# SunYangtian/Splatter_A_Video

Measured on AMD Instinct MI355X. Metric: rendered frames/sec fwd+bwd @480p, 300k Gaussians, higher is better.
Workload: dtype f32

## Files before the change

include/splat_hip.h:

```cpp
#ifndef SPLAT_HIP_H
#define SPLAT_HIP_H

#include <stddef.h>
#include <stdint.h>

#ifdef __cplusplus
extern "C" {
#endif

typedef void *splat_stream_t;

#define SPLAT_OK 0
#define SPLAT_E_ARG (-1)
#define SPLAT_E_LAUNCH (-2)
#define SPLAT_E_CAPACITY (-3)

const char *splat_last_error(void);
#define SPLAT_ABI_VERSION 22
int splat_abi_version(void);
const char *splat_build_id(void);
void splat_set_deterministic(int on);
int splat_get_deterministic(void);
int splat_fill_f32(float *dst, size_t n, float value, splat_stream_t stream);
int splat_set_option(const char *key, int value);
// ... 175 lines not shown
                                         float nearest, float extent, float *uv, float *depth, float *conic,
                                         int32_t *radius, splat_stream_t stream);
int splat_bin_count_batch(int F, int P, const float *uv, const int32_t *radius, int W, int H, void *scratch,
                          int32_t *tile_range, int32_t *M_out, splat_stream_t stream);
int splat_bin_sort_batch(int F, int P, const float *uv, const float *depth, const int32_t *radius, int W, int H,
                         void *scratch, int32_t *tile_range, int64_t capacity, uint64_t *keys, int32_t *idx_sorted,
                         int32_t *overflow_out, int32_t *goff_incl , int32_t *owner, int32_t *slot_sorted,
                         splat_stream_t stream);
int splat_bin_count_batch_reach(int F, int P, const float *uv, const int32_t *radius, const float *conic,
                                const float *opacity, int64_t opacity_frame_stride, int W, int H, void *scratch,
                                int32_t *tile_range, int32_t *M_out, int32_t *gcount, uint32_t *reach, splat_stream_t stream);
int splat_bin_sort_batch_reach(int F, int P, const float *uv, const float *depth, const int32_t *radius, const uint32_t *reach,
                               int W, int H, void *scratch, int32_t *tile_range, int64_t capacity, uint64_t *keys,
                               int32_t *idx_sorted, int32_t *overflow_out, int32_t *goff_incl , int32_t *owner,
                               int32_t *slot_sorted, splat_stream_t stream);
int splat_alpha_blending_forward_batch(int F, int P, int C, const float *uv, const float *conic, const float *opacity,
                                       int64_t opacity_frame_stride, const float *feature, int64_t feature_frame_stride,
                                       const int32_t *idx_sorted, const int32_t *tile_range, int64_t capacity, float bg,
                                       const float *bg_channels, int W, int H, int K, int enable_truncation, float *out,
                                       float *final_T, int32_t *ncontrib, int32_t *gs_idx, float *pack_scratch,
                                       uint32_t *cull_flags , splat_stream_t stream);
size_t splat_blend_pair_stride(int C, int want_abs, int has_bias);
int splat_alpha_blending_backward_batch(int F, int P, int C, const int32_t *idx_sorted, const int32_t *tile_range,
                                        int64_t capacity, float bg, int W, int H, const float *final_T,
                                        const int32_t *ncontrib, const float *dL_dout, int want_abs,
                                        const int32_t *slot_sorted, float *pair_records, const float *pack,
                                        const uint32_t *cull_flags ,
                                        float *dbg_T_front , splat_stream_t stream);
int splat_frames_gauss_backward_static(int F, int P, int C, int W, int H, int64_t capacity, int want_abs,
                                       const float *pair_records, const int32_t *goff_incl, const int32_t *radius,
                                       const float *xyz, const float *scales, const float *uquats, const float *extr,
                                       int accumulate, float *d_xyz, float *d_scales, float *d_uquats, float *d_opacity,
                                       float *d_feature, float *tap, float *abs_tap, int32_t *radii_max,
                                       splat_stream_t stream);

typedef struct splat_camera_t {
// ... 249 lines not shown
```

splatter_a_video_amd/_lib.py:

```python
from __future__ import annotations

import ctypes
import os
from typing import Optional

import torch

_HERE = os.path.dirname(os.path.abspath(__file__))
LIB_PATH = os.environ.get("SPLAT_LIB_PATH") or os.path.join(_HERE, "libsplat_hip.so")
_lib: Optional[ctypes.CDLL] = None

ABI_VERSION = 22

SYMBOLS = [
    "splat_last_error", "splat_abi_version", "splat_build_id", "splat_set_deterministic", "splat_get_deterministic",
    "splat_fill_f32", "splat_set_option", "splat_get_option",
    "splat_project_point_forward", "splat_project_point_backward",
    "splat_compute_cov3d_forward", "splat_compute_cov3d_backward",
    "splat_ewa_project_forward", "splat_ewa_project_backward",
    "splat_compute_sh_forward", "splat_compute_sh_backward",
    "splat_bin_scratch_bytes", "splat_bin_count", "splat_bin_sort",
    "splat_compute_gaussian_key", "splat_compute_tile_gaussian_range",
    "splat_alpha_blending_forward", "splat_alpha_blending_backward", "splat_alpha_blending_forward_flags",
    "splat_alpha_blending_backward_flags", "splat_blend_pair_floats", "splat_blend_pack_floats",
# ... 13 lines not shown
    "splat_frames_gauss_backward_static", "splat_alpha_blending_backward_batch_set", "splat_frames_gauss_backward_static_set",
    "splat_blend_sets_pair_stride", "splat_blend_sets_pack_floats", "splat_alpha_blending_backward_batch_sets",
    "splat_alpha_blending_forward_batch_sets", "splat_pair_records_segment_sum", "splat_alpha_blending_backward_batch_sets_packed",
    "splat_frames_gauss_backward_static_sets", "splat_frames_gauss_backward_dynamic_sets",
    "splat_preprocess_forward_batch_cam", "splat_frames_gauss_backward_static_cam", "splat_frames_gauss_backward_static_sets_cam",
    "splat_preprocess_persp_forward", "splat_preprocess_persp_backward",
    "splat_alpha_blending_forward_batch_sources", "splat_frames_gauss_backward_dynamic_sources",
    "splat_frames_gauss_backward_static_sources_cam", "splat_blend_sets_uses_forward_pack",
    "splat_dynamic_positions_batch_forward", "splat_dynamic_positions_batch_backward",
    "splat_arap_energy_batch", "splat_knn_brute_scratch_bytes", "splat_knn_brute_batch", "splat_l1_loss_grad",
    "splat_alpha_blending_backward_batch_sets_l1", "splat_bin_count_batch_reach", "splat_bin_sort_batch_reach",
    "splat_profile_enable", "splat_profile_reset", "splat_profile_read",
    "splat_ssim_scratch_bytes", "splat_ssim_forward", "splat_ssim_backward", "splat_dssim_l1_loss_grad",
    "splat_track_loss_scratch_bytes", "splat_track_loss_grad",
    "splat_depth_dpt_scratch_bytes", "splat_depth_stats", "splat_depth_dpt_loss_grad",
]


class SplatError(RuntimeError):
    pass


_raw_stream = getattr(torch._C, "_cuda_getCurrentRawStream", None)
_cur_device = getattr(torch._C, "_cuda_getDevice", None)


def lib() -> ctypes.CDLL:
    global _lib
    if _lib is None:
        if not os.path.exists(LIB_PATH):
# ... 147 lines not shown
```

splatter_a_video_amd/csrc/binning.hip:

```cpp
#include "common.h"
#include <cstdlib>

#define BIN_BLOCK 256
#define BIN_MAX_NB 512
#define BIN_CHUNK 512
#define BIN_CHUNK_BATCH 2048
#define BIN_BATCH_FRAMES 4
#define BIN_LDS_TILES 12288
#define BIN_GLOBAL_BLOCKS 2048
#define SORT_BLOCK 256
#define SORT_LDS_KEYS 2048

struct BinPlan {
    int T, gx, gy;
    int NB;
    int chunk;
    bool lds;
    int nchunk;
    size_t off_matrix, off_tilecount, off_total, off_chunksum;
    size_t bytes;
};

static inline int imax(int a, int b) { return a > b ? a : b; }
static inline int imin(int a, int b) { return a < b ? a : b; }
// ... 48 lines not shown
__device__ __forceinline__ int reach_cell_shift(int w, int h) {
    int sh = 1;
    while ((((w - 1) >> sh) + 1) * (((h - 1) >> sh) + 1) > 31) ++sh;
    return sh;
}
__device__ __forceinline__ int reach_big_count(unsigned word, int w, int h) {
    const int sh = reach_cell_shift(w, h), c = 1 << sh, ncx = ((w - 1) >> sh) + 1, ncy = ((h - 1) >> sh) + 1;
    int n = 0;
    unsigned bit = 1u;
    for (int cy = 0; cy < ncy; ++cy)
        for (int cx = 0; cx < ncx; ++cx, bit <<= 1)
            if (word & bit) n += imin_(c, w - cx * c) * imin_(c, h - cy * c);
    return n;
}

template <bool LDS>
__global__ void __launch_bounds__(BIN_BLOCK)
bin_count_kernel(int P, const float2 *__restrict__ uv, const int *__restrict__ radius, int gx, int gy, int T,
                 int chunk, int *__restrict__ matrix, int *__restrict__ gcount, int *__restrict__ chunk_sum,
                 long long S, const float *__restrict__ conic, const float *__restrict__ opacity, long long opacity_fs,
                 unsigned *__restrict__ reach) {
    extern __shared__ __attribute__((aligned(16))) int cnt[];
    __shared__ int wave_pairs[BIN_BLOCK / 64];
    const int wg = blockIdx.x;
    {
        const size_t f = blockIdx.y;
        uv += f * P; radius += f * P; matrix += f * S; chunk_sum += f * S;
        if (gcount) gcount += f * P;
        if (reach) { conic += f * 3 * (size_t)P; opacity += f * (size_t)opacity_fs; reach += f * P; }
    }
    int pairs = 0;
    if (LDS) {
        for (int t = threadIdx.x; t < T; t += BIN_BLOCK) cnt[t] = 0;
        __syncthreads();
    }
    const int beg = wg * chunk, end = imin_(P, beg + chunk);
    for (int i = beg + threadIdx.x; i < end; i += BIN_BLOCK) {
        const int r = radius[i];
        if (r <= 0) {
            if (gcount) gcount[i] = 0;
            if (reach) reach[i] = 0u;
            continue;
        }
        const float2 q = uv[i];
        int x0, y0, x1, y1;
        tile_rect(q.x, q.y, r, gx, gy, x0, y0, x1, y1);
        const int area = (x1 - x0) * (y1 - y0);
        if (reach) {
            const float cA = conic[3 * (size_t)i], cB = conic[3 * (size_t)i + 1], cC = conic[3 * (size_t)i + 2], o = opacity[i];
            unsigned word;
            int kept = 0;
            if (area < 32) {
                const CullP cp = cull_params(cA, cB, cC, o);
                unsigned m = 0u, bit = 1u;
                for (int ty = y0; ty < y1; ++ty)
                    for (int tx = x0; tx < x1; ++tx, bit <<= 1) {
                        const float fx = (float)(tx * TILE), fy = (float)(ty * TILE);
                        if (cull_test(q.x, q.y, cA, cB, cC, cp, fx, fx + (float)(TILE - 1), fy, fy + (float)(TILE - 1))) {
                            m |= bit;
                            if (LDS) atomicAdd(&cnt[ty * gx + tx], 1);
                            else atomicAdd(&matrix[ty * gx + tx], 1);
                        }
                    }
                kept = __popc(m);
                word = m;
            } else {
// ... 555 lines not shown
                idx_sorted[r0 + i] = id;
            } else {
                idx_sorted[r0 + i] = (int)lo;
            }
        }
    }
}

extern "C" size_t splat_bin_scratch_bytes(int P, int W, int H) {
    if (P < 0 || W <= 0 || H <= 0) return 0;
    return make_plan(P, W, H).bytes;
}

static int bin_count_impl(int F, int P, const float *uv, const int32_t *radius, int W, int H, void *scratch,
                          int32_t *tile_range, int32_t *M_out, int32_t *gcount, hipStream_t s, const float *conic = nullptr,
                          const float *opacity = nullptr, long long opacity_fs = 0, uint32_t *reach = nullptr) {
    const BinPlan p = make_plan(P, W, H, F);
    const long long S = (long long)(p.bytes / sizeof(int));
    char *base = (char *)scratch;
    int *matrix = (int *)(base + p.off_matrix);
    int *tile_count = (int *)(base + p.off_tilecount);
    int *total = (int *)(base + p.off_total);
    int *chunk_sum = (int *)(base + p.off_chunksum);
    if (p.lds) {
        SPLAT_LAUNCH("bin_count", bin_count_kernel<true>, dim3(p.NB, F), dim3(BIN_BLOCK), (size_t)p.T * sizeof(int), s,
                     P, (const float2 *)uv, radius, p.gx, p.gy, p.T, p.chunk, matrix, gcount, chunk_sum, S, conic, opacity, opacity_fs,
                     reach);
    } else {
        for (int f = 0; f < F; ++f)
            SPLAT_CHECK_HIP(hipMemsetAsync(matrix + (size_t)f * S, 0, (size_t)p.T * sizeof(int), s));
        const int nblk = p.nchunk;
        const int chunk = (P + nblk - 1) / nblk;
        SPLAT_LAUNCH("bin_count", bin_count_kernel<false>, dim3(nblk, F), dim3(BIN_BLOCK), 0, s, P, (const float2 *)uv,
                     radius, p.gx, p.gy, p.T, chunk > 0 ? chunk : 1, matrix, gcount, chunk_sum, S, conic, opacity, opacity_fs, reach);
    }
    SPLAT_POST_LAUNCH();
    if (p.lds) {
        SPLAT_LAUNCH("bin_colscan", bin_colscan_kernel, dim3((p.T + COLSCAN_COLS - 1) / COLSCAN_COLS, F),
                     dim3(COLSCAN_COLS * COLSCAN_GROUPS), 0, s, p.T, p.NB, matrix, tile_count, S);
        SPLAT_POST_LAUNCH();
    } else {
        for (int f = 0; f < F; ++f)
            SPLAT_CHECK_HIP(hipMemcpyAsync(tile_count + (size_t)f * S, matrix + (size_t)f * S, (size_t)p.T * sizeof(int),
                                           hipMemcpyDeviceToDevice, s));
    }
    SPLAT_LAUNCH("bin_tilescan", bin_tilescan_kernel, dim3(1, F), dim3(1024), 0, s, p.T, tile_count, tile_range, M_out, total,
                 p.nchunk, chunk_sum, S);
    SPLAT_POST_LAUNCH();
    return SPLAT_OK;
}
// ... 71 lines not shown
    return bin_sort_impl(F, P, uv, depth, radius, W, H, scratch, tile_range, capacity, keys, idx_sorted, overflow_out,
                         goff_incl, owner_scratch, slot_sorted, (hipStream_t)stream);
}


extern "C" int splat_bin_count_batch_reach(int F, int P, const float *uv, const int32_t *radius, const float *conic,
                                           const float *opacity, int64_t opacity_frame_stride, int W, int H, void *scratch,
                                           int32_t *tile_range, int32_t *M_out, int32_t *gcount, uint32_t *reach,
                                           splat_stream_t stream) {
    SPLAT_CHECK_ARG(F >= 1 && F <= 65535 && P >= 1 && W > 0 && H > 0 && opacity_frame_stride >= 0, "bad sizes");
    SPLAT_CHECK_ARG(scratch && tile_range && uv && radius && conic && opacity && reach, "null pointer");
    return bin_count_impl(F, P, uv, radius, W, H, scratch, tile_range, M_out, gcount, (hipStream_t)stream, conic, opacity,
                          (long long)opacity_frame_stride, reach);
}

extern "C" int splat_bin_sort_batch_reach(int F, int P, const float *uv, const float *depth, const int32_t *radius,
                                          const uint32_t *reach, int W, int H, void *scratch, int32_t *tile_range,
                                          int64_t capacity, uint64_t *keys, int32_t *idx_sorted, int32_t *overflow_out,
                                          int32_t *goff_incl, int32_t *owner_scratch, int32_t *slot_sorted,
                                          splat_stream_t stream) {
    SPLAT_CHECK_ARG(F >= 1 && F <= 65535 && P >= 1 && W > 0 && H > 0 && capacity >= 1, "bad sizes");
    SPLAT_CHECK_ARG(scratch && tile_range && overflow_out && uv && depth && radius && keys && idx_sorted && goff_incl &&
                        owner_scratch && slot_sorted && reach,
                    "null pointer");
    return bin_sort_impl(F, P, uv, depth, radius, W, H, scratch, tile_range, capacity, keys, idx_sorted, overflow_out,
                         goff_incl, owner_scratch, slot_sorted, (hipStream_t)stream, reach);
}


__global__ void __launch_bounds__(256)
// ... 59 lines not shown
```

splatter_a_video_amd/csrc/blend.hip:

```cpp
#include <stdlib.h>

#include <utility>

#include "common.h"

__device__ __forceinline__ float exp2_guard(float pw, bool &ok) {
    ok = true;
    return __builtin_amdgcn_fmed3f(__builtin_amdgcn_exp2f(pw), 0.f, 1.f);
}

struct BlendArgs {
    int P, C;
    int c0, cn;
    const float2 *uv;
    const float *conic;
    const float *opacity;
    const float *feature;
    const float *bias;
    const int *idx_sorted;
    const int2 *tile_range;
    float bg;
    const float *bgc;
    int W, H, gx;
    int K, trunc;
// ... 92 lines not shown
    pw = __builtin_fmaf(xx, c0.w, pw);
    pw = __builtin_fmaf(xy, c1.x, pw);
    return __builtin_fmaf(yy, c1.y, pw);
}
__device__ __forceinline__ float neg_power_factored(float dx, float dy, float cA, float cB, float cC) {
#pragma clang fp contract(off)
    const float h = __builtin_fmaf(cA, 0.5f * dx, cB * dy);
    return __builtin_fmaf(dx, h, (cC * (0.5f * dy)) * dy);
}
__device__ __forceinline__ float exp_neg(float q) { return __builtin_amdgcn_exp2f(-BLEND_L2E * q); }

struct __attribute__((packed, aligned(4))) F3 {
    float x, y, z;
};

template <int CH>
struct Rec {
    static constexpr int RS = (8 + CH + 15) & ~15;
    static constexpr int RQ = RS / 4;
    static constexpr int CULL = (RS - 8 - CH >= 5) ? RS - 5 : -1;
};


template <bool SETS = false>
__device__ __forceinline__ void stage_feature_rows(float *s_rec, int LS, int at, const float *src, int cn, int i0, int nrec) {
    if (!src || cn <= 0) return;
    const float *p = src + (size_t)i0 * cn;
    for (int e = threadIdx.x; e < nrec * cn; e += 256) {
        const int row = e / cn, ch = e - row * cn;
        s_rec[row * LS + (SETS ? 8 + 8 * ((at + ch) & 3) + ((at + ch) >> 2) : at + ch)] = p[e];
    }
}

template <int CH, bool BIAS, bool EXACT>
__global__ void __launch_bounds__(256)
pack_kernel(const BlendArgs B) {
    const BlendArgs A = frame_args(B, blockIdx.y);
    constexpr int RS = Rec<CH>::RS, RQ = Rec<CH>::RQ;
    constexpr int LS = RS + 4;
    __shared__ __attribute__((aligned(16))) float s_rec[256 * LS];
    const int i0 = blockIdx.x * 256;
    const int i = i0 + threadIdx.x;
    float r[RS];
#pragma unroll
    for (int k = 0; k < RS; ++k) r[k] = 0.f;
    if (i < A.P) {
        const float2 q = A.uv[i];
        r[0] = q.x; r[1] = q.y;
        r[2] = A.conic[3 * i]; r[3] = A.conic[3 * i + 1]; r[4] = A.conic[3 * i + 2];
        r[5] = A.opacity[i];
        if (BIAS) r[6] = A.bias[i];
        r[7] = __int_as_float(i);
        if (A.feature) {
            const float *f = A.feature + (size_t)i * A.C + A.c0;
#pragma unroll
            for (int k = 0; k < CH; ++k)
                if (EXACT || k < A.cn) r[8 + k] = f[k];
        }
        if (Rec<CH>::CULL >= 0) {
            constexpr int CO = Rec<CH>::CULL >= 0 ? Rec<CH>::CULL : 0;
            const CullP cp = cull_params(r[2], r[3], r[4], r[5]);
            r[CO] = cp.hx; r[CO + 1] = cp.hy; r[CO + 2] = cp.tauq; r[CO + 3] = cp.ia; r[CO + 4] = cp.ic;
        }
    }
    {
        float4 *row = reinterpret_cast<float4 *>(s_rec + threadIdx.x * LS);
#pragma unroll
        for (int k = 0; k < RS; k += 4) row[k / 4] = make_float4(r[k], r[k + 1], r[k + 2], r[k + 3]);
        __syncthreads();
        const int nrec = imin_(256, A.P - i0);
        if (!A.feature) {
            for (int sidx = 0; sidx < B.nsrc; ++sidx)
                stage_feature_rows(s_rec, LS, 8 + B.src_c0[sidx] - B.c0, B.src_f[sidx] + (size_t)blockIdx.y * B.src_fs[sidx],
                                   B.src_cn[sidx], i0, nrec);
            __syncthreads();
        }
        float4 *dst = reinterpret_cast<float4 *>(A.pack + (size_t)i0 * RS);
        for (int c = threadIdx.x; c < nrec * RQ; c += 256) {
// ... 3235 lines not shown
template <int CH>
static int launch_pack(const BlendArgs &A, bool bias, hipStream_t s) {
    if (A.P == 0) return SPLAT_OK;
    const dim3 grid((unsigned)((A.P + 255) / 256), (unsigned)A.F), block(256);
    const bool exact = A.cn == CH;
    if (bias) { if (exact) SPLAT_LAUNCH("blend_pack", (pack_kernel<CH, true, true>), grid, block, 0, s, A); else SPLAT_LAUNCH("blend_pack", (pack_kernel<CH, true, false>), grid, block, 0, s, A); }
    else { if (exact) SPLAT_LAUNCH("blend_pack", (pack_kernel<CH, false, true>), grid, block, 0, s, A); else SPLAT_LAUNCH("blend_pack", (pack_kernel<CH, false, false>), grid, block, 0, s, A); }
    SPLAT_POST_LAUNCH();
    return SPLAT_OK;
}

template <int CH>
static int launch_fwd(const BlendArgs &A, int T, bool enh, bool bias, hipStream_t s) {
    const dim3 grid((unsigned)(T * A.F)), block(256);
    const bool exact = A.cn == CH;
    {
        const int rc = launch_pack<CH>(A, bias, s);
        if (rc != SPLAT_OK) return rc;
    }
#define FWD(E, B, X) SPLAT_LAUNCH("blend_fwd", (blend_fwd_kernel<CH, E, B, X>), grid, block, 0, s, A)
    if (enh) {
        if (bias) { if (exact) FWD(true, true, true); else FWD(true, true, false); }
        else { if (exact) FWD(true, false, true); else FWD(true, false, false); }
    } else {
        if (bias) { if (exact) FWD(false, true, true); else FWD(false, true, false); }
        else { if (exact) FWD(false, false, true); else FWD(false, false, false); }
    }
#undef FWD
    SPLAT_POST_LAUNCH();
    return SPLAT_OK;
}
// ... 35 lines not shown
        SPLAT_POST_LAUNCH();
    }
    return SPLAT_OK;
}

template <int CH>
static int launch_bwd(const BlendArgs &A, int T, bool bias, bool pair, hipStream_t s) {
    if (!A.pack_valid) {
        const int rc = launch_pack<CH>(A, bias, s);
        if (rc != SPLAT_OK) return rc;
    }
    const bool abs_ = A.dL_dabs_uv != nullptr;
    if (abs_) return bias ? launch_bwd_ab<CH, true, true>(A, T, pair, s) : launch_bwd_ab<CH, true, false>(A, T, pair, s);
    return bias ? launch_bwd_ab<CH, false, true>(A, T, pair, s) : launch_bwd_ab<CH, false, false>(A, T, pair, s);
}

static inline int chunk_ch(int cn) { return cn <= 1 ? 1 : cn <= 3 ? 3 : cn <= 8 ? 8 : cn <= 16 ? 16 : cn <= 20 ? 20 : cn <= 24 ? 24 : 32; }

static int fwd_chunk(const BlendArgs &A, int T, bool enh, bool bias, hipStream_t s) {
    switch (chunk_ch(A.cn)) {
        case 1: return launch_fwd<1>(A, T, enh, bias, s);
        case 3: return launch_fwd<3>(A, T, enh, bias, s);
        case 8: return launch_fwd<8>(A, T, enh, bias, s);
        case 16: return launch_fwd<16>(A, T, enh, bias, s);
        case 20: return launch_fwd<20>(A, T, enh, bias, s);
        case 24: return launch_fwd<24>(A, T, enh, bias, s);
        default: return launch_fwd<32>(A, T, enh, bias, s);
    }
}

static int bwd_chunk(const BlendArgs &A, int T, bool bias, bool pair, hipStream_t s) {
    switch (chunk_ch(A.cn)) {
// ... 144 lines not shown
                                                   const int32_t *slot_sorted, float *pair_scratch, float *pack_scratch,
                                                   int pack_is_valid, float *dbg_T_front, const uint32_t *cull_flags,
                                                   splat_stream_t stream) {
    return blend_backward_impl(P, C, uv, conic, opacity, feature, opacity_bias, idx_sorted, tile_range, bg, W, H, final_T, ncontrib,
                               dL_dout, dL_duv, dL_dabs_uv, dL_dconic, dL_dopacity, dL_dfeature, dL_dopacity_bias, dL_dndc,
                               dL_dabs_ndc, goff_incl, slot_sorted, pair_scratch, pack_scratch, pack_is_valid, dbg_T_front,
                               cull_flags, stream);
}


extern "C" size_t splat_blend_pair_stride(int C, int want_abs, int has_bias) {
    const int ng = 6 + (want_abs ? 2 : 0) + (has_bias ? 1 : 0);
    return (size_t)PAIR_STRIDE(ng + chunk_ch(C > 32 ? 32 : C));
}

extern "C" int splat_alpha_blending_forward_batch(int F, int P, int C, const float *uv, const float *conic,
                                                  const float *opacity, int64_t opacity_frame_stride,
                                                  const float *feature, int64_t feature_frame_stride,
                                                  const int32_t *idx_sorted, const int32_t *tile_range, int64_t capacity,
                                                  float bg, const float *bg_channels, int W, int H, int K,
                                                  int enable_truncation, float *out, float *final_T, int32_t *ncontrib,
                                                  int32_t *gs_idx, float *pack_scratch, uint32_t *cull_flags,
                                                  splat_stream_t stream) {
    SPLAT_CHECK_ARG(F >= 1 && P >= 1 && C >= 1 && C <= 32 && W > 0 && H > 0 && capacity >= 1, "bad sizes (C <= 32)");
    SPLAT_CHECK_ARG(uv && conic && opacity && feature && idx_sorted && tile_range && out && final_T && ncontrib &&
                        pack_scratch,
                    "null pointer");
    const bool enh = (gs_idx != nullptr) && K > 0;
    BlendArgs A;
    memset(&A, 0, sizeof(A));
    A.P = P; A.C = C;
    A.uv = (const float2 *)uv; A.conic = conic; A.opacity = opacity; A.feature = feature;
    A.idx_sorted = idx_sorted; A.tile_range = (const int2 *)tile_range;
    A.bg = bg; A.bgc = bg_channels; A.W = W; A.H = H; A.gx = (W + TILE - 1) / TILE;
    A.K = enh ? K : 0; A.trunc = enable_truncation ? 1 : 0;
    A.out = out; A.final_T = final_T; A.ncontrib = ncontrib; A.gs_idx = gs_idx;
    A.pack = pack_scratch;
    A.cull_flags = cull_flags;
    const int T = A.gx * ((H + TILE - 1) / TILE);
    SPLAT_CHECK_ARG((long long)F * T < (1ll << 31), "too many tiles");
    A.F = F; A.T = T; A.cap = capacity;
    A.pack_fs = (long long)P * (long long)splat_blend_pack_floats(C);
    A.opacity_fs = opacity_frame_stride; A.feature_fs = feature_frame_stride;
    A.c0 = 0; A.cn = C;
    return fwd_chunk(A, T, enh, false, (hipStream_t)stream);
}

extern "C" int splat_alpha_blending_forward_batch_sources(int F, int P, int C, int nsrc, const splat_feature_source_t *src,
                                                          const float *uv, const float *conic, const float *opacity,
                                                          int64_t opacity_frame_stride, const int32_t *idx_sorted,
                                                          const int32_t *tile_range, int64_t capacity,
                                                          const float *bg_channels, int W, int H, int K, int enable_truncation,
                                                          float *out, float *final_T, int32_t *ncontrib, int32_t *gs_idx,
                                                          float *pack_scratch, uint32_t *cull_flags, splat_stream_t stream) {
    SPLAT_CHECK_ARG(F >= 1 && P >= 1 && C >= 1 && C <= 32 && W > 0 && H > 0 && capacity >= 1, "bad sizes (C <= 32)");
    SPLAT_CHECK_ARG(src && nsrc >= 1 && nsrc <= SPLAT_MAX_SOURCES && bg_channels, "null / oversized source table");
    SPLAT_CHECK_ARG(uv && conic && opacity && idx_sorted && tile_range && out && final_T && ncontrib && pack_scratch, "null pointer");
    BlendArgs A;
    memset(&A, 0, sizeof(A));
    {
// ... 324 lines not shown
```

splatter_a_video_amd/csrc/common.h:

```cpp
#pragma once
#include <hip/hip_runtime.h>
#include <stdint.h>
#include <stdio.h>
#include <string.h>

#include "../../include/splat_hip.h"

#define TILE 16
#define TILE_PIX 256
#define WAVE 64

void splat_set_error(const char *fmt, ...);

#define SPLAT_CHECK_ARG(cond, msg)                     \
    do {                                               \
        if (!(cond)) {                                 \
            splat_set_error("%s: %s", __func__, msg);  \
            return SPLAT_E_ARG;                        \
        }                                              \
    } while (0)

#define SPLAT_CHECK_HIP(expr)                                                          \
    do {                                                                               \
        hipError_t e_ = (expr);                                                        \
// ... 87 lines not shown
    const float t = 255.f * o;
    if (t < 0.999f) {
        p.hx = -1.f;
        return p;
    }
    const float det = a * c - b * b;
    if (!(det > 0.f) || !(a > 0.f) || !(c > 0.f)) return p;
    const float relerr = 4e-7f * (a * c + b * b) / det;
    if (!(relerr < 0.25f)) return p;
    const float tau0 = fmaxf(2.f * __logf(t), 0.f);
    const float tau = tau0 * (1.f + 2.f * relerr) * 1.002f + 2e-3f;
    const float inv = 1.f / det;
    p.hx = sqrtf(tau * c * inv) * 1.001f + 0.01f;
    p.hy = sqrtf(tau * a * inv) * 1.001f + 0.01f;
    p.tauq = tau * 1.002f + 2e-3f;
    p.ia = 1.f / a;
    p.ic = 1.f / c;
    return p;
}

__device__ __forceinline__ bool cull_test(float u, float v, float a, float b, float c, const CullP &p, float bx0,
                                          float bx1, float by0, float by1) {
    const float dx0 = bx0 - u, dx1 = bx1 - u, dy0 = by0 - v, dy1 = by1 - v;
    const float ddx = fmaxf(fmaxf(dx0, -dx1), 0.f);
    const float ddy = fmaxf(fmaxf(dy0, -dy1), 0.f);
    if (!((ddx <= p.hx) && (ddy <= p.hy))) return false;
    if (ddx == 0.f && ddy == 0.f) return true;
    const float INF = __builtin_inff();
    const float xe = dx0 > 0.f ? dx0 : dx1, ye = dy0 > 0.f ? dy0 : dy1;
    const float ys = fminf(fmaxf(-b * xe * p.ic, dy0), dy1), xs = fminf(fmaxf(-b * ye * p.ia, dx0), dx1);
    const float qx = a * xe * xe + 2.f * b * xe * ys + c * ys * ys;
    const float qy = a * xs * xs + 2.f * b * xs * ye + c * ye * ye;
    const float qmin = fminf(ddx > 0.f ? qx : INF, ddy > 0.f ? qy : INF);
    const float r2 = fmaxf(dx0 * dx0, dx1 * dx1) + fmaxf(dy0 * dy0, dy1 * dy1);
    const float qerr = 4e-6f * (a + c + 2.f * fabsf(b)) * r2;
    return qmin <= p.tauq + qerr;
}

template <bool ABS, bool BIAS>
struct GradLayout {
    static constexpr int NG = 6 + (ABS ? 2 : 0) + (BIAS ? 1 : 0);
    static constexpr int I_ABS = 6;
    static constexpr int I_BIAS = 6 + (ABS ? 2 : 0);
};
#define PAIR_STRIDE(nc) (((nc) + 3) & ~3)
constexpr int SETS_NG = 12;
constexpr int XCD_RUN = 64;
__device__ __forceinline__ int xcd_tile(int b, int T) {
    constexpr int S = XCD_RUN;
    const int full = (T / (8 * S)) * (8 * S);
    if (b >= full) return b;
    const int x = b & 7, q = b >> 3;
    return ((q / S) * 8 + x) * S + (q % S);
// ... 4 lines not shown
```

splatter_a_video_amd/csrc/frames.hip:

```cpp
#include "common.h"

static splat_camera_t batch_camera(const splat_frames_t *b) {
    splat_camera_t cam;
    memset(&cam, 0, sizeof(cam));
    cam.perspective = b->perspective; cam.intr = b->intr; cam.intr_frame_stride = b->intr_frame_stride;
    cam.extr = b->extr; cam.extr_frame_stride = b->extr_frame_stride; cam.offsets = b->offsets;
    return cam;
}

static int frames_bin_count(const splat_frames_t *b) {
    if (b->reach) {
        SPLAT_CHECK_ARG(b->opacity != nullptr, "reach masks need the opacity");
        return splat_bin_count_batch_reach(b->F, b->P, b->uv, b->radius, b->conic, b->opacity, 0, b->W, b->H, b->bin_scratch,
                                           b->tile_range, b->pairs, nullptr, b->reach, b->stream);
    }
    return splat_bin_count_batch(b->F, b->P, b->uv, b->radius, b->W, b->H, b->bin_scratch, b->tile_range, b->pairs, b->stream);
}

extern "C" int splat_frames_forward(const splat_frames_t *b) {
    SPLAT_CHECK_ARG(b != nullptr && b->struct_bytes == sizeof(splat_frames_t), "splat_frames_t of another ABI version");
    SPLAT_CHECK_ARG(b->capacity >= 1, "capacity (pairs reserved per frame) must be set: run splat_frames_count first");
    const splat_camera_t cam = batch_camera(b);
    int rc = splat_preprocess_forward_batch_cam(b->F, b->P, b->xyz, b->offsets, b->scales, b->uquats, &cam, b->W, b->H,
                                                b->nearest, b->extent, b->uv, b->depth, b->conic, b->radius, b->stream);
    if (rc != SPLAT_OK) return rc;
    rc = frames_bin_count(b);
    if (rc != SPLAT_OK) return rc;
    if (b->reach)
        rc = splat_bin_sort_batch_reach(b->F, b->P, b->uv, b->depth, b->radius, b->reach, b->W, b->H, b->bin_scratch,
                                        b->tile_range, b->capacity, b->keys, b->idx_sorted, b->overflow, b->goff_incl, b->owner,
                                        b->slot_sorted, b->stream);
    else
        rc = splat_bin_sort_batch(b->F, b->P, b->uv, b->depth, b->radius, b->W, b->H, b->bin_scratch, b->tile_range, b->capacity,
                                  b->keys, b->idx_sorted, b->overflow, b->goff_incl, b->owner, b->slot_sorted, b->stream);
    if (rc != SPLAT_OK) return rc;
    return splat_alpha_blending_forward_batch(b->F, b->P, b->C, b->uv, b->conic, b->opacity, 0, b->feature, 0, b->idx_sorted,
                                              b->tile_range, b->capacity, b->bg, nullptr, b->W, b->H, 0, 0, b->out, b->final_T,
                                              b->ncontrib, nullptr, b->pack, b->cull_flags, b->stream);
}

extern "C" int splat_frames_count(const splat_frames_t *b) {
    SPLAT_CHECK_ARG(b != nullptr && b->struct_bytes == sizeof(splat_frames_t), "splat_frames_t of another ABI version");
    const splat_camera_t cam = batch_camera(b);
    int rc = splat_preprocess_forward_batch_cam(b->F, b->P, b->xyz, b->offsets, b->scales, b->uquats, &cam, b->W, b->H,
                                                b->nearest, b->extent, b->uv, b->depth, b->conic, b->radius, b->stream);
    if (rc != SPLAT_OK) return rc;
    return frames_bin_count(b);
}

extern "C" int splat_frames_backward(const splat_frames_t *b) {
// ... 18 lines not shown
```

splatter_a_video_amd/frames.py:

```python
from __future__ import annotations

import ctypes
import os
import warnings
from typing import Dict, Optional

import torch
from torch import Tensor

from . import _lib as L
from .gs.fused_ops import check_sink
from .gs.point_ops import _extr12, _points


_FRAMES_FIELDS = ([("struct_bytes", ctypes.c_size_t)]
                  + [(n, ctypes.c_int32) for n in ("F", "P", "W", "H", "C", "want_abs", "accumulate")]
                  + [("capacity", ctypes.c_int64)] + [(n, ctypes.c_float) for n in ("nearest", "extent", "bg")]
                  + [("stream", ctypes.c_void_p)]
                  + [(n, ctypes.c_void_p) for n in (
                      "xyz", "offsets", "scales", "uquats", "opacity", "feature", "extr", "uv", "depth", "conic", "radius",
                      "bin_scratch", "tile_range", "pairs", "overflow", "goff_incl", "owner", "idx_sorted", "slot_sorted", "keys",
                      "pack", "out", "final_T", "ncontrib", "dL_dout", "pair_records", "d_xyz", "d_scales", "d_uquats",
                      "d_opacity", "d_feature", "tap", "abs_tap", "radii_max", "dbg_T_front", "cull_flags")]
                  + [("extr_frame_stride", ctypes.c_int64), ("intr_frame_stride", ctypes.c_int64), ("intr", ctypes.c_void_p),
# ... 175 lines not shown
                "forward has overwritten the buffers this backward reads (sorted lists, packed records, final_T, ncontrib).  "
                "A FrameBatch holds ONE forward at a time: run the backward before the next render* (also under no_grad), or "
                "use one FrameBatch per micro-batch.")

    def memory_bytes(self) -> int:
        return sum(t.numel() * t.element_size() for t in vars(self).values() if isinstance(t, Tensor))

    def _geometry(self, xyz, scales, uquats, offsets, cam: "_Camera", nearest, extent, opacity=None, op_fs=0):
        lib, st = L.lib(), L.stream()
        F_, P_, W, H = self.F, self.P, self.W, self.H
        L.check(lib.splat_preprocess_forward_batch_cam(
            L.ci(F_), L.ci(P_), L.ptr(xyz), L.ptr(offsets), L.ptr(scales), L.ptr(uquats), ctypes.byref(cam.struct()), L.ci(W),
            L.ci(H), L.cf(nearest), L.cf(extent), L.ptr(self.uv), L.ptr(self.depth), L.ptr(self.conic), L.ptr(self.radius), st))
        self._bin_and_sort(opacity, op_fs)

    def _bin_and_sort(self, opacity: Optional[Tensor] = None, op_fs: int = 0):
        lib, st = L.lib(), L.stream()
        F_, P_, W, H = self.F, self.P, self.W, self.H
        reach = opacity is not None and OPTIONS["reach"]
        if reach:
            L.check(lib.splat_bin_count_batch_reach(
                L.ci(F_), L.ci(P_), L.ptr(self.uv), L.ptr(self.radius), L.ptr(self.conic), L.ptr(opacity), ctypes.c_int64(op_fs),
                L.ci(W), L.ci(H), L.ptr(self.bin_scratch), L.ptr(self.tile_range), L.ptr(self.pairs), L.ptr(None),
                L.ptr(self.reach), st))
        else:
            L.check(lib.splat_bin_count_batch(L.ci(F_), L.ci(P_), L.ptr(self.uv), L.ptr(self.radius), L.ci(W), L.ci(H),
                                              L.ptr(self.bin_scratch), L.ptr(self.tile_range), L.ptr(self.pairs), st))
        if self.capacity is None:
            self._reserve(int(int(self.pairs.max().item()) * self.slack) + 1024)
        cap = self.capacity
        if reach:
            L.check(lib.splat_bin_sort_batch_reach(
                L.ci(F_), L.ci(P_), L.ptr(self.uv), L.ptr(self.depth), L.ptr(self.radius), L.ptr(self.reach), L.ci(W), L.ci(H),
                L.ptr(self.bin_scratch), L.ptr(self.tile_range),
                ctypes.c_int64(cap), L.ptr(self.keys), L.ptr(self.idx_sorted), L.ptr(self.overflow), L.ptr(self.goff),
                L.ptr(self.owner), L.ptr(self.slot_sorted), st))
        else:
            L.check(lib.splat_bin_sort_batch(
                L.ci(F_), L.ci(P_), L.ptr(self.uv), L.ptr(self.depth), L.ptr(self.radius), L.ci(W), L.ci(H),
                L.ptr(self.bin_scratch), L.ptr(self.tile_range), ctypes.c_int64(cap), L.ptr(self.keys), L.ptr(self.idx_sorted),
                L.ptr(self.overflow), L.ptr(self.goff), L.ptr(self.owner), L.ptr(self.slot_sorted), st))
        self._note_overflow()

    def _struct(self, xyz, scales, uquats, opacity, feature, offsets, cam, bg, nearest=0.01, extent=1.3) -> _SplatFrames:
        b = _SplatFrames()
        extr = cam.extr
        b.extr_frame_stride, b.intr_frame_stride = cam.extr_fs, cam.intr_fs
        b.intr = None if cam.intr is None else cam.intr.data_ptr()
        b.perspective = 1 if cam.perspective else 0
        b.struct_bytes = ctypes.sizeof(_SplatFrames)
        b.F, b.P, b.W, b.H, b.C = self.F, self.P, self.W, self.H, self.C
        b.want_abs = 1 if self.want_abs else 0
        b.capacity = self.capacity or 0
        b.nearest, b.extent, b.bg = nearest, extent, bg
        b.stream = L.stream()
        dp = lambda t: None if t is None else t.data_ptr()
        for name, t in dict(xyz=xyz, offsets=offsets, scales=scales, uquats=uquats, opacity=opacity, feature=feature, extr=extr,
# ... 139 lines not shown
        feature = _points(feature, "feature", fb.C)
        rot_poly, rot_fourier = L.need(rot_poly, "rot_poly_feat"), L.need(rot_fourier, "rot_fourier_feat")
        if cubic.numel() != P * 4 * I * 3 or rot_poly.numel() != P * 16 or rot_fourier.numel() != P * 32 or opacity.numel() != P:
            raise ValueError("parameter shapes do not match the batch (P Gaussians, I spline segments)")
        if position.shape[0] != P or rotation.shape[0] != P or scaling.shape[0] != P or feature.shape[0] != P:
            raise ValueError(f"the batch was built for {P} Gaussians")
        extr_c = _extr12(extr)
        lib, st = L.lib(), L.stream()
        W, H, C = fb.W, fb.H, fb.C
        ctx.gen = fb._begin_forward()
        opa_t = torch.empty(P, 1, dtype=torch.float32, device=fb.dev)
        L.check(lib.splat_frame_preprocess_forward_batch(
            L.ci(F), L.ci(P), L.ci(I), L.ptr(tab), L.ptr(position), L.ptr(cubic), L.ci(layout), L.ptr(rotation), L.ptr(rot_poly),
            L.ptr(rot_fourier), L.ptr(opacity), L.ptr(scaling), L.ptr(extr_c), L.ci(W), L.ci(H), L.cf(nearest), L.cf(extent),
            L.ptr(fb.uv), L.ptr(fb.depth), L.ptr(fb.conic), L.ptr(fb.radius), L.ptr(opa_t), st))
        fb._bin_and_sort(opa_t)
        cap = fb.capacity
        out = torch.empty(F, C, H, W, dtype=torch.float32, device=fb.dev)
        L.check(lib.splat_alpha_blending_forward_batch(
            L.ci(F), L.ci(P), L.ci(C), L.ptr(fb.uv), L.ptr(fb.conic), L.ptr(opa_t), ctypes.c_int64(0), L.ptr(feature),
            ctypes.c_int64(0), L.ptr(fb.idx_sorted), L.ptr(fb.tile_range), ctypes.c_int64(cap), L.cf(bg), L.ptr(None), L.ci(W),
            L.ci(H), L.ci(0), L.ci(0), L.ptr(out), L.ptr(fb.final_T), L.ptr(fb.ncontrib), L.ptr(None), L.ptr(fb.pack),
            L.ptr(fb.cull_flags), st))
        ctx.fb, ctx.meta, ctx.sink = fb, (I, layout, bg), sink
        ctx.save_for_backward(position, cubic, rotation, opacity, scaling, feature, rot_poly, rot_fourier, extr_c, tab)
        return out

    @staticmethod
    def backward(ctx, dL_dout):
        fb: FrameBatch = ctx.fb
        fb._check_generation(ctx.gen)
        position, cubic, rotation, opacity, scaling, feature, rot_poly, rot_fourier, extr_c, tab = ctx.saved_tensors
        I, layout, bg = ctx.meta
        sink = ctx.sink or {}
# ... 565 lines not shown
```

Before: 5380.

## Fuse blend record packing into the bin count pass

The bin count kernel now writes each Gaussian's 16-float blend record (uv, conic, opacity, id, features, cull params) while it already has those values loaded, so the forward blend can skip its separate pack kernel launch and reread. A new packed entry point and a pack_valid flag let the blend forward use the prefilled buffer when the channel count is at most 8 and reach masks are enabled. It adds register pressure and store traffic to the count kernel, and introduces a separately written cull-parameter function that must match the original one exactly.

```diff
diff --git a/include/splat_hip.h b/include/splat_hip.h
--- a/include/splat_hip.h
+++ b/include/splat_hip.h
@@ -213,12 +213,22 @@
                                int W, int H, void *scratch, int32_t *tile_range, int64_t capacity, uint64_t *keys,
                                int32_t *idx_sorted, int32_t *overflow_out, int32_t *goff_incl , int32_t *owner,
                                int32_t *slot_sorted, splat_stream_t stream);
+int splat_bin_count_batch_reach_pack(int F, int P, const float *uv, const int32_t *radius, const float *conic,
+                                     const float *opacity, int64_t opacity_frame_stride, const float *feature,
+                                     int64_t feature_frame_stride, int C, int W, int H, void *scratch, int32_t *tile_range,
+                                     int32_t *M_out, int32_t *gcount, uint32_t *reach, float *pack, splat_stream_t stream);
 int splat_alpha_blending_forward_batch(int F, int P, int C, const float *uv, const float *conic, const float *opacity,
                                        int64_t opacity_frame_stride, const float *feature, int64_t feature_frame_stride,
                                        const int32_t *idx_sorted, const int32_t *tile_range, int64_t capacity, float bg,
                                        const float *bg_channels, int W, int H, int K, int enable_truncation, float *out,
                                        float *final_T, int32_t *ncontrib, int32_t *gs_idx, float *pack_scratch,
                                        uint32_t *cull_flags , splat_stream_t stream);
+int splat_alpha_blending_forward_batch_packed(int F, int P, int C, const float *uv, const float *conic, const float *opacity,
+                                              int64_t opacity_frame_stride, const float *feature, int64_t feature_frame_stride,
+                                              const int32_t *idx_sorted, const int32_t *tile_range, int64_t capacity, float bg,
+                                              const float *bg_channels, int W, int H, int K, int enable_truncation, float *out,
+                                              float *final_T, int32_t *ncontrib, int32_t *gs_idx, float *pack_scratch,
+                                              uint32_t *cull_flags, splat_stream_t stream);
 size_t splat_blend_pair_stride(int C, int want_abs, int has_bias);
 int splat_alpha_blending_backward_batch(int F, int P, int C, const int32_t *idx_sorted, const int32_t *tile_range,
                                         int64_t capacity, float bg, int W, int H, const float *final_T,
diff --git a/splatter_a_video_amd/_lib.py b/splatter_a_video_amd/_lib.py
--- a/splatter_a_video_amd/_lib.py
+++ b/splatter_a_video_amd/_lib.py
@@ -51,6 +51,7 @@
     "splat_ssim_scratch_bytes", "splat_ssim_forward", "splat_ssim_backward", "splat_dssim_l1_loss_grad",
     "splat_track_loss_scratch_bytes", "splat_track_loss_grad",
     "splat_depth_dpt_scratch_bytes", "splat_depth_stats", "splat_depth_dpt_loss_grad",
+    "splat_bin_count_batch_reach_pack", "splat_alpha_blending_forward_batch_packed",
 ]
 
 
diff --git a/splatter_a_video_amd/csrc/binning.hip b/splatter_a_video_amd/csrc/binning.hip
--- a/splatter_a_video_amd/csrc/binning.hip
+++ b/splatter_a_video_amd/csrc/binning.hip
@@ -86,12 +86,31 @@
     return n;
 }
 
-template <bool LDS>
-__global__ void __launch_bounds__(BIN_BLOCK)
+template <int CH>
+__device__ __forceinline__ void count_store_record(float *__restrict__ rec, float u, float v, float cA, float cB, float cC, float o,
+                                                   int id, const float *__restrict__ frow, int cn) {
+    static_assert(Rec<CH>::RS == 16, "the count pass writes 16-float records");
+    float fr[CH], r[16];
+    constexpr int SURE = CH == 8 ? 4 : CH == 3 ? 2 : 1;
+#pragma unroll
+    for (int k = 0; k < CH; ++k) fr[k] = frow[(k < SURE || k < cn) ? k : 0];
+#pragma unroll
+    for (int k = 0; k < 16; ++k) r[k] = 0.f;
+    CullP cp;
+    if (Rec<CH>::CULL >= 0) cp = cull_params_rec(cA, cB, cC, o);
+    rec_fill<CH, false>(r, u, v, cA, cB, cC, o, id, fr, cn, cp);
+    float4 *dst = reinterpret_cast<float4 *>(rec);
+#pragma unroll
+    for (int k = 0; k < 4; ++k) dst[k] = make_float4(r[4 * k], r[4 * k + 1], r[4 * k + 2], r[4 * k + 3]);
+}
+
+template <bool LDS, int PCH = 0>
+__global__ void __launch_bounds__(BIN_BLOCK) __attribute__((amdgpu_num_sgpr(96)))
 bin_count_kernel(int P, const float2 *__restrict__ uv, const int *__restrict__ radius, int gx, int gy, int T,
                  int chunk, int *__restrict__ matrix, int *__restrict__ gcount, int *__restrict__ chunk_sum,
                  long long S, const float *__restrict__ conic, const float *__restrict__ opacity, long long opacity_fs,
-                 unsigned *__restrict__ reach) {
+                 unsigned *__restrict__ reach, float *__restrict__ pack = nullptr, long long pack_fs = 0,
+                 const float *__restrict__ feature = nullptr, long long feature_fs = 0, int C = 0) {
     extern __shared__ __attribute__((aligned(16))) int cnt[];
     __shared__ int wave_pairs[BIN_BLOCK / 64];
     const int wg = blockIdx.x;
@@ -100,6 +119,7 @@
         uv += f * P; radius += f * P; matrix += f * S; chunk_sum += f * S;
         if (gcount) gcount += f * P;
         if (reach) { conic += f * 3 * (size_t)P; opacity += f * (size_t)opacity_fs; reach += f * P; }
+        if (PCH > 0) { pack += f * (size_t)pack_fs; feature += f * (size_t)feature_fs; }
     }
     int pairs = 0;
     if (LDS) {
@@ -122,6 +142,7 @@
             const float cA = conic[3 * (size_t)i], cB = conic[3 * (size_t)i + 1], cC = conic[3 * (size_t)i + 2], o = opacity[i];
             unsigned word;
             int kept = 0;
+            if (PCH > 0) count_store_record<PCH ? PCH : 1>(pack + 16 * (size_t)i, q.x, q.y, cA, cB, cC, o, i, feature + (size_t)i * C, C);
             if (area < 32) {
                 const CullP cp = cull_params(cA, cB, cC, o);
                 unsigned m = 0u, bit = 1u;
@@ -707,26 +728,32 @@
 
 static int bin_count_impl(int F, int P, const float *uv, const int32_t *radius, int W, int H, void *scratch,
                           int32_t *tile_range, int32_t *M_out, int32_t *gcount, hipStream_t s, const float *conic = nullptr,
-                          const float *opacity = nullptr, long long opacity_fs = 0, uint32_t *reach = nullptr) {
+                          const float *opacity = nullptr, long long opacity_fs = 0, uint32_t *reach = nullptr,
+                          float *pack = nullptr, const float *feature = nullptr, long long feature_fs = 0, int C = 0) {
     const BinPlan p = make_plan(P, W, H, F);
+    const long long pack_fs = 16ll * P;
     const long long S = (long long)(p.bytes / sizeof(int));
     char *base = (char *)scratch;
     int *matrix = (int *)(base + p.off_matrix);
     int *tile_count = (int *)(base + p.off_tilecount);
     int *total = (int *)(base + p.off_total);
     int *chunk_sum = (int *)(base + p.off_chunksum);
-    if (p.lds) {
-        SPLAT_LAUNCH("bin_count", bin_count_kernel<true>, dim3(p.NB, F), dim3(BIN_BLOCK), (size_t)p.T * sizeof(int), s,
-                     P, (const float2 *)uv, radius, p.gx, p.gy, p.T, p.chunk, matrix, gcount, chunk_sum, S, conic, opacity, opacity_fs,
-                     reach);
-    } else {
+    const int nblk = p.lds ? p.NB : p.nchunk;
+    const int chunk = p.lds ? p.chunk : imax(1, (P + nblk - 1) / nblk);
+    if (!p.lds)
         for (int f = 0; f < F; ++f)
             SPLAT_CHECK_HIP(hipMemsetAsync(matrix + (size_t)f * S, 0, (size_t)p.T * sizeof(int), s));
-        const int nblk = p.nchunk;
-        const int chunk = (P + nblk - 1) / nblk;
-        SPLAT_LAUNCH("bin_count", bin_count_kernel<false>, dim3(nblk, F), dim3(BIN_BLOCK), 0, s, P, (const float2 *)uv,
-                     radius, p.gx, p.gy, p.T, chunk > 0 ? chunk : 1, matrix, gcount, chunk_sum, S, conic, opacity, opacity_fs, reach);
-    }
+#define BIN_COUNT(LDS_, PCH_)                                                                                                     \
+    SPLAT_LAUNCH("bin_count", (bin_count_kernel<LDS_, PCH_>), dim3(nblk, F), dim3(BIN_BLOCK), LDS_ ? (size_t)p.T * sizeof(int) : 0, \
+                 s, P, (const float2 *)uv, radius, p.gx, p.gy, p.T, chunk, matrix, gcount, chunk_sum, S, conic, opacity,           \
+                 opacity_fs, reach, pack, pack_fs, feature, feature_fs, C)
+    switch (pack ? chunk_ch(C) : 0) {
+        case 0: if (p.lds) BIN_COUNT(true, 0); else BIN_COUNT(false, 0); break;
+        case 1: if (p.lds) BIN_COUNT(true, 1); else BIN_COUNT(false, 1); break;
+        case 3: if (p.lds) BIN_COUNT(true, 3); else BIN_COUNT(false, 3); break;
+        default: if (p.lds) BIN_COUNT(true, 8); else BIN_COUNT(false, 8); break;
+    }
+#undef BIN_COUNT
     SPLAT_POST_LAUNCH();
     if (p.lds) {
         SPLAT_LAUNCH("bin_colscan", bin_colscan_kernel, dim3((p.T + COLSCAN_COLS - 1) / COLSCAN_COLS, F),
@@ -828,6 +855,19 @@
                           (long long)opacity_frame_stride, reach);
 }
 
+extern "C" int splat_bin_count_batch_reach_pack(int F, int P, const float *uv, const int32_t *radius, const float *conic,
+                                                const float *opacity, int64_t opacity_frame_stride, const float *feature,
+                                                int64_t feature_frame_stride, int C, int W, int H, void *scratch,
+                                                int32_t *tile_range, int32_t *M_out, int32_t *gcount, uint32_t *reach,
+                                                float *pack, splat_stream_t stream) {
+    SPLAT_CHECK_ARG(F >= 1 && F <= 65535 && P >= 1 && W > 0 && H > 0 && opacity_frame_stride >= 0 && feature_frame_stride >= 0,
+                    "bad sizes");
+    SPLAT_CHECK_ARG(C >= 1 && C <= 8, "the count pass packs rows of at most 8 channels");
+    SPLAT_CHECK_ARG(scratch && tile_range && uv && radius && conic && opacity && reach && feature && pack, "null pointer");
+    return bin_count_impl(F, P, uv, radius, W, H, scratch, tile_range, M_out, gcount, (hipStream_t)stream, conic, opacity,
+                          (long long)opacity_frame_stride, reach, pack, feature, (long long)feature_frame_stride, C);
+}
+
 extern "C" int splat_bin_sort_batch_reach(int F, int P, const float *uv, const float *depth, const int32_t *radius,
                                           const uint32_t *reach, int W, int H, void *scratch, int32_t *tile_range,
                                           int64_t capacity, uint64_t *keys, int32_t *idx_sorted, int32_t *overflow_out,
diff --git a/splatter_a_video_amd/csrc/blend.hip b/splatter_a_video_amd/csrc/blend.hip
--- a/splatter_a_video_amd/csrc/blend.hip
+++ b/splatter_a_video_amd/csrc/blend.hip
@@ -130,12 +130,6 @@
     float x, y, z;
 };
 
-template <int CH>
-struct Rec {
-    static constexpr int RS = (8 + CH + 15) & ~15;
-    static constexpr int RQ = RS / 4;
-    static constexpr int CULL = (RS - 8 - CH >= 5) ? RS - 5 : -1;
-};
 
 
 template <bool SETS = false>
@@ -162,22 +156,11 @@
     for (int k = 0; k < RS; ++k) r[k] = 0.f;
     if (i < A.P) {
         const float2 q = A.uv[i];
-        r[0] = q.x; r[1] = q.y;
-        r[2] = A.conic[3 * i]; r[3] = A.conic[3 * i + 1]; r[4] = A.conic[3 * i + 2];
-        r[5] = A.opacity[i];
+        const float cA = A.conic[3 * i], cB = A.conic[3 * i + 1], cC = A.conic[3 * i + 2], o = A.opacity[i];
+        CullP cp;
+        if (Rec<CH>::CULL >= 0) cp = cull_params_rec(cA, cB, cC, o);
+        rec_fill<CH, EXACT>(r, q.x, q.y, cA, cB, cC, o, i, A.feature ? A.feature + (size_t)i * A.C + A.c0 : nullptr, A.cn, cp);
         if (BIAS) r[6] = A.bias[i];
-        r[7] = __int_as_float(i);
-        if (A.feature) {
-            const float *f = A.feature + (size_t)i * A.C + A.c0;
-#pragma unroll
-            for (int k = 0; k < CH; ++k)
-                if (EXACT || k < A.cn) r[8 + k] = f[k];
-        }
-        if (Rec<CH>::CULL >= 0) {
-            constexpr int CO = Rec<CH>::CULL >= 0 ? Rec<CH>::CULL : 0;
-            const CullP cp = cull_params(r[2], r[3], r[4], r[5]);
-            r[CO] = cp.hx; r[CO + 1] = cp.hy; r[CO + 2] = cp.tauq; r[CO + 3] = cp.ia; r[CO + 4] = cp.ic;
-        }
     }
     {
         float4 *row = reinterpret_cast<float4 *>(s_rec + threadIdx.x * LS);
@@ -3443,7 +3426,7 @@
 static int launch_fwd(const BlendArgs &A, int T, bool enh, bool bias, hipStream_t s) {
     const dim3 grid((unsigned)(T * A.F)), block(256);
     const bool exact = A.cn == CH;
-    {
+    if (!A.pack_valid) {
         const int rc = launch_pack<CH>(A, bias, s);
         if (rc != SPLAT_OK) return rc;
     }
@@ -3509,8 +3492,6 @@
     if (abs_) return bias ? launch_bwd_ab<CH, true, true>(A, T, pair, s) : launch_bwd_ab<CH, true, false>(A, T, pair, s);
     return bias ? launch_bwd_ab<CH, false, true>(A, T, pair, s) : launch_bwd_ab<CH, false, false>(A, T, pair, s);
 }
-
-static inline int chunk_ch(int cn) { return cn <= 1 ? 1 : cn <= 3 ? 3 : cn <= 8 ? 8 : cn <= 16 ? 16 : cn <= 20 ? 20 : cn <= 24 ? 24 : 32; }
 
 static int fwd_chunk(const BlendArgs &A, int T, bool enh, bool bias, hipStream_t s) {
     switch (chunk_ch(A.cn)) {
@@ -3685,7 +3666,7 @@
     return (size_t)PAIR_STRIDE(ng + chunk_ch(C > 32 ? 32 : C));
 }
 
-extern "C" int splat_alpha_blending_forward_batch(int F, int P, int C, const float *uv, const float *conic,
+static int blend_forward_batch_impl(int pack_valid, int F, int P, int C, const float *uv, const float *conic,
                                                   const float *opacity, int64_t opacity_frame_stride,
                                                   const float *feature, int64_t feature_frame_stride,
                                                   const int32_t *idx_sorted, const int32_t *tile_range, int64_t capacity,
@@ -3706,7 +3687,7 @@
     A.bg = bg; A.bgc = bg_channels; A.W = W; A.H = H; A.gx = (W + TILE - 1) / TILE;
     A.K = enh ? K : 0; A.trunc = enable_truncation ? 1 : 0;
     A.out = out; A.final_T = final_T; A.ncontrib = ncontrib; A.gs_idx = gs_idx;
-    A.pack = pack_scratch;
+    A.pack = pack_scratch; A.pack_valid = pack_valid;
     A.cull_flags = cull_flags;
     const int T = A.gx * ((H + TILE - 1) / TILE);
     SPLAT_CHECK_ARG((long long)F * T < (1ll << 31), "too many tiles");
@@ -3715,6 +3696,33 @@
     A.opacity_fs = opacity_frame_stride; A.feature_fs = feature_frame_stride;
     A.c0 = 0; A.cn = C;
     return fwd_chunk(A, T, enh, false, (hipStream_t)stream);
+}
+
+extern "C" int splat_alpha_blending_forward_batch(int F, int P, int C, const float *uv, const float *conic,
+                                                  const float *opacity, int64_t opacity_frame_stride,
+                                                  const float *feature, int64_t feature_frame_stride,
+                                                  const int32_t *idx_sorted, const int32_t *tile_range, int64_t capacity,
+                                                  float bg, const float *bg_channels, int W, int H, int K,
+                                                  int enable_truncation, float *out, float *final_T, int32_t *ncontrib,
+                                                  int32_t *gs_idx, float *pack_scratch, uint32_t *cull_flags,
+                                                  splat_stream_t stream) {
+    return blend_forward_batch_impl(0, F, P, C, uv, conic, opacity, opacity_frame_stride, feature, feature_frame_stride, idx_sorted,
+                                   tile_range, capacity, bg, bg_channels, W, H, K, enable_truncation, out, final_T, ncontrib, gs_idx,
+                                   pack_scratch, cull_flags, stream);
+}
+
+extern "C" int splat_alpha_blending_forward_batch_packed(int F, int P, int C, const float *uv, const float *conic,
+                                                  const float *opacity, int64_t opacity_frame_stride,
+                                                  const float *feature, int64_t feature_frame_stride,
+                                                  const int32_t *idx_sorted, const int32_t *tile_range, int64_t capacity,
+                                                  float bg, const float *bg_channels, int W, int H, int K,
+                                                  int enable_truncation, float *out, float *final_T, int32_t *ncontrib,
+                                                  int32_t *gs_idx, float *pack_scratch, uint32_t *cull_flags,
+                                                  splat_stream_t stream) {
+    SPLAT_CHECK_ARG(C >= 1 && C <= 8, "the count pass packs rows of at most 8 channels");
+    return blend_forward_batch_impl(1, F, P, C, uv, conic, opacity, opacity_frame_stride, feature, feature_frame_stride, idx_sorted,
+                                   tile_range, capacity, bg, bg_channels, W, H, K, enable_truncation, out, final_T, ncontrib, gs_idx,
+                                   pack_scratch, cull_flags, stream);
 }
 
 extern "C" int splat_alpha_blending_forward_batch_sources(int F, int P, int C, int nsrc, const splat_feature_source_t *src,
diff --git a/splatter_a_video_amd/csrc/common.h b/splatter_a_video_amd/csrc/common.h
--- a/splatter_a_video_amd/csrc/common.h
+++ b/splatter_a_video_amd/csrc/common.h
@@ -125,6 +125,32 @@
     p.hx = sqrtf(tau * c * inv) * 1.001f + 0.01f;
     p.hy = sqrtf(tau * a * inv) * 1.001f + 0.01f;
     p.tauq = tau * 1.002f + 2e-3f;
+    p.ia = 1.f / a;
+    p.ic = 1.f / c;
+    return p;
+}
+
+__device__ __forceinline__ CullP cull_params_rec(float a, float b, float c, float o) {
+#pragma clang fp contract(off)
+    CullP p;
+    const float INF = __builtin_inff();
+    p.hx = INF; p.hy = INF; p.tauq = INF; p.ia = 0.f; p.ic = 0.f;
+    const float t = 255.f * o;
+    if (t < 0.999f) {
+        p.hx = -1.f;
+        return p;
+    }
+    const float bb = b * b;
+    const float det = __builtin_fmaf(a, c, -bb);
+    if (!(det > 0.f) || !(a > 0.f) || !(c > 0.f)) return p;
+    const float relerr = 4e-7f * (a * c + bb) / det;
+    if (!(relerr < 0.25f)) return p;
+    const float tau0 = fmaxf(2.f * __logf(t), 0.f);
+    const float tau = __builtin_fmaf(tau0 * __builtin_fmaf(2.f, relerr, 1.f), 1.002f, 2e-3f);
+    const float inv = 1.f / det;
+    p.hx = __builtin_fmaf(sqrtf(tau * c * inv), 1.001f, 0.01f);
+    p.hy = __builtin_fmaf(sqrtf(tau * a * inv), 1.001f, 0.01f);
+    p.tauq = __builtin_fmaf(tau, 1.002f, 2e-3f);
     p.ia = 1.f / a;
     p.ic = 1.f / c;
     return p;
@@ -148,6 +174,33 @@
     return qmin <= p.tauq + qerr;
 }
 
+template <int CH>
+struct Rec {
+    static constexpr int RS = (8 + CH + 15) & ~15;
+    static constexpr int RQ = RS / 4;
+    static constexpr int CULL = (RS - 8 - CH >= 5) ? RS - 5 : -1;
+};
+
+static inline int chunk_ch(int cn) { return cn <= 1 ? 1 : cn <= 3 ? 3 : cn <= 8 ? 8 : cn <= 16 ? 16 : cn <= 20 ? 20 : cn <= 24 ? 24 : 32; }
+
+template <int CH, bool EXACT>
+__device__ __forceinline__ void rec_fill(float (&r)[Rec<CH>::RS], float u, float v, float cA, float cB, float cC, float o, int id,
+                                         const float *__restrict__ f, int cn, const CullP &cp) {
+    r[0] = u; r[1] = v;
+    r[2] = cA; r[3] = cB; r[4] = cC;
+    r[5] = o;
+    r[7] = __int_as_float(id);
+    if (f) {
+#pragma unroll
+        for (int k = 0; k < CH; ++k)
+            if (EXACT || k < cn) r[8 + k] = f[k];
+    }
+    if (Rec<CH>::CULL >= 0) {
+        constexpr int CO = Rec<CH>::CULL >= 0 ? Rec<CH>::CULL : 0;
+        r[CO] = cp.hx; r[CO + 1] = cp.hy; r[CO + 2] = cp.tauq; r[CO + 3] = cp.ia; r[CO + 4] = cp.ic;
+    }
+}
+
 template <bool ABS, bool BIAS>
 struct GradLayout {
     static constexpr int NG = 6 + (ABS ? 2 : 0) + (BIAS ? 1 : 0);
diff --git a/splatter_a_video_amd/csrc/frames.hip b/splatter_a_video_amd/csrc/frames.hip
--- a/splatter_a_video_amd/csrc/frames.hip
+++ b/splatter_a_video_amd/csrc/frames.hip
@@ -8,9 +8,17 @@
     return cam;
 }
 
-static int frames_bin_count(const splat_frames_t *b) {
+static bool frames_count_packs(const splat_frames_t *b) {
+    return b->reach && b->pack && b->feature && b->C <= 8;
+}
+
+static int frames_bin_count(const splat_frames_t *b, bool pack = false) {
     if (b->reach) {
         SPLAT_CHECK_ARG(b->opacity != nullptr, "reach masks need the opacity");
+        if (pack)
+            return splat_bin_count_batch_reach_pack(b->F, b->P, b->uv, b->radius, b->conic, b->opacity, 0, b->feature, 0, b->C, b->W,
+                                                    b->H, b->bin_scratch, b->tile_range, b->pairs, nullptr, b->reach, b->pack,
+                                                    b->stream);
         return splat_bin_count_batch_reach(b->F, b->P, b->uv, b->radius, b->conic, b->opacity, 0, b->W, b->H, b->bin_scratch,
                                            b->tile_range, b->pairs, nullptr, b->reach, b->stream);
     }
@@ -24,7 +32,8 @@
     int rc = splat_preprocess_forward_batch_cam(b->F, b->P, b->xyz, b->offsets, b->scales, b->uquats, &cam, b->W, b->H,
                                                 b->nearest, b->extent, b->uv, b->depth, b->conic, b->radius, b->stream);
     if (rc != SPLAT_OK) return rc;
-    rc = frames_bin_count(b);
+    const bool packed = frames_count_packs(b);
+    rc = frames_bin_count(b, packed);
     if (rc != SPLAT_OK) return rc;
     if (b->reach)
         rc = splat_bin_sort_batch_reach(b->F, b->P, b->uv, b->depth, b->radius, b->reach, b->W, b->H, b->bin_scratch,
@@ -34,6 +43,10 @@
         rc = splat_bin_sort_batch(b->F, b->P, b->uv, b->depth, b->radius, b->W, b->H, b->bin_scratch, b->tile_range, b->capacity,
                                   b->keys, b->idx_sorted, b->overflow, b->goff_incl, b->owner, b->slot_sorted, b->stream);
     if (rc != SPLAT_OK) return rc;
+    if (packed)
+        return splat_alpha_blending_forward_batch_packed(b->F, b->P, b->C, b->uv, b->conic, b->opacity, 0, b->feature, 0,
+                                                         b->idx_sorted, b->tile_range, b->capacity, b->bg, nullptr, b->W, b->H, 0, 0,
+                                                         b->out, b->final_T, b->ncontrib, nullptr, b->pack, b->cull_flags, b->stream);
     return splat_alpha_blending_forward_batch(b->F, b->P, b->C, b->uv, b->conic, b->opacity, 0, b->feature, 0, b->idx_sorted,
                                               b->tile_range, b->capacity, b->bg, nullptr, b->W, b->H, 0, 0, b->out, b->final_T,
                                               b->ncontrib, nullptr, b->pack, b->cull_flags, b->stream);
diff --git a/splatter_a_video_amd/frames.py b/splatter_a_video_amd/frames.py
--- a/splatter_a_video_amd/frames.py
+++ b/splatter_a_video_amd/frames.py
@@ -213,11 +213,18 @@
             L.ci(H), L.cf(nearest), L.cf(extent), L.ptr(self.uv), L.ptr(self.depth), L.ptr(self.conic), L.ptr(self.radius), st))
         self._bin_and_sort(opacity, op_fs)
 
-    def _bin_and_sort(self, opacity: Optional[Tensor] = None, op_fs: int = 0):
+    def _bin_and_sort(self, opacity: Optional[Tensor] = None, op_fs: int = 0, feature: Optional[Tensor] = None,
+                      feat_fs: int = 0) -> bool:
         lib, st = L.lib(), L.stream()
         F_, P_, W, H = self.F, self.P, self.W, self.H
         reach = opacity is not None and OPTIONS["reach"]
-        if reach:
+        packed = reach and feature is not None and self.C <= 8
+        if packed:
+            L.check(lib.splat_bin_count_batch_reach_pack(
+                L.ci(F_), L.ci(P_), L.ptr(self.uv), L.ptr(self.radius), L.ptr(self.conic), L.ptr(opacity), ctypes.c_int64(op_fs),
+                L.ptr(feature), ctypes.c_int64(feat_fs), L.ci(self.C), L.ci(W), L.ci(H), L.ptr(self.bin_scratch),
+                L.ptr(self.tile_range), L.ptr(self.pairs), L.ptr(None), L.ptr(self.reach), L.ptr(self.pack), st))
+        elif reach:
             L.check(lib.splat_bin_count_batch_reach(
                 L.ci(F_), L.ci(P_), L.ptr(self.uv), L.ptr(self.radius), L.ptr(self.conic), L.ptr(opacity), ctypes.c_int64(op_fs),
                 L.ci(W), L.ci(H), L.ptr(self.bin_scratch), L.ptr(self.tile_range), L.ptr(self.pairs), L.ptr(None),
@@ -240,6 +247,7 @@
                 L.ptr(self.bin_scratch), L.ptr(self.tile_range), ctypes.c_int64(cap), L.ptr(self.keys), L.ptr(self.idx_sorted),
                 L.ptr(self.overflow), L.ptr(self.goff), L.ptr(self.owner), L.ptr(self.slot_sorted), st))
         self._note_overflow()
+        return packed
 
     def _struct(self, xyz, scales, uquats, opacity, feature, offsets, cam, bg, nearest=0.01, extent=1.3) -> _SplatFrames:
         b = _SplatFrames()
@@ -409,10 +417,11 @@
             L.ci(F), L.ci(P), L.ci(I), L.ptr(tab), L.ptr(position), L.ptr(cubic), L.ci(layout), L.ptr(rotation), L.ptr(rot_poly),
             L.ptr(rot_fourier), L.ptr(opacity), L.ptr(scaling), L.ptr(extr_c), L.ci(W), L.ci(H), L.cf(nearest), L.cf(extent),
             L.ptr(fb.uv), L.ptr(fb.depth), L.ptr(fb.conic), L.ptr(fb.radius), L.ptr(opa_t), st))
-        fb._bin_and_sort(opa_t)
+        packed = fb._bin_and_sort(opa_t, 0, feature, 0)
         cap = fb.capacity
         out = torch.empty(F, C, H, W, dtype=torch.float32, device=fb.dev)
-        L.check(lib.splat_alpha_blending_forward_batch(
+        blend = lib.splat_alpha_blending_forward_batch_packed if packed else lib.splat_alpha_blending_forward_batch
+        L.check(blend(
             L.ci(F), L.ci(P), L.ci(C), L.ptr(fb.uv), L.ptr(fb.conic), L.ptr(opa_t), ctypes.c_int64(0), L.ptr(feature),
             ctypes.c_int64(0), L.ptr(fb.idx_sorted), L.ptr(fb.tile_range), ctypes.c_int64(cap), L.cf(bg), L.ptr(None), L.ci(W),
             L.ci(H), L.ci(0), L.ci(0), L.ptr(out), L.ptr(fb.final_T), L.ptr(fb.ncontrib), L.ptr(None), L.ptr(fb.pack),
```

New measurement: 5282. -1.8%, worse.
